# vressegu/sdeflow-light

Measured on AMD Instinct MI355X. Metric: score-matching train steps/sec (+ reverse-SDE sample steps/sec), higher is better.
Workload: dtype f32

## Files before the change

sdeflow_light_amd/csrc/conv_kernels.hip:

```cpp
#include "common.h"
#include <algorithm>
#include <type_traits>
#include <stdlib.h>

#define CONV_MAX_SRC 2

struct ConvGeom {
  int N, Hi, Wi, Ho, Wo;
  int KH, KW, strideH, padH, strideW, padW;
  int mode;
  int ups;
};

struct ConvArgs {
  ConvGeom g;
  const float* src[CONV_MAX_SRC];
  int C[CONV_MAX_SRC];
  int koff[CONV_MAX_SRC];
  int nsrc;
  const float* Wp;
  int Cout, CoutP, Ktot;
  const float* bias;
  const float* samp_bias;
  int n_bias, n_samp;
// ... 1126 lines not shown
  tile_origin<16, 16>(tile, tiles_x, tiles_y, n, y0, x0);
  auto stage = [&](int s_, int c0) __attribute__((always_inline)) {
    f32x4 st[H18_NST], ga, gb;
    unsigned valid;
    halo18_load(A, g, A.src[s_], A.C[s_], up, c0, (size_t)n * ctot_all + (s_ ? A.C[0] : 0), n, y0, x0, tid, st, valid, ga, gb);
    halo18_store(A, cur, tid, st, valid, ga, gb);
  };

  const size_t a_co_stride = (size_t)16 * A.Ktot, pos_stride = (size_t)A.CoutP * A.Ktot;
  if constexpr (WL) {
    static_assert(NCO == 2, "the LDS weight image is laid out for two output-channel tiles");
    float* wbuf = cw_lds + halo * CT_P;
    auto ngrp_of = [&](int s_, int c_) { const int rem = A.C[s_] - c_ * CT_KC; return rem >= CT_KC ? 2 : ((rem + 15) >> 4); };
    auto wfill = [&](int s_, int c_, int g_, int half, int b) __attribute__((always_inline)) {
      wino_wfill(A.Wp + (size_t)(co0 + il) * A.Ktot + A.koff[s_] + c_ * CT_KC + 16 * g_ + 4 * q + (size_t)(8 * half) * pos_stride,
                 wbuf + b * 4096, w, pos_stride, a_co_stride);
    };
    int cs = 0, cc = 0, grp = 0, step = 0;
    wfill(0, 0, 0, 0, 0);
    for (;;) {
      if (grp == 0) {
        asm volatile("s_waitcnt lgkmcnt(0)\n\ts_barrier" ::: "memory");
        stage(cs, cc * CT_KC);
      }
      int ns = cs, nc = cc, ng = grp + 1;
      bool more = true;
      if (ng >= ngrp_of(cs, cc)) {
        ng = 0; ++nc;
        if (nc >= nch[cs]) { nc = 0; ++ns; more = ns < A.nsrc; }
      }
      f32x4 d[4][4];
#pragma unroll
      for (int half = 0; half < 2; ++half) {
        asm volatile("s_waitcnt vmcnt(0) lgkmcnt(0)\n\ts_barrier" ::: "memory");
        if (half == 0) wfill(cs, cc, grp, 1, (step + 1) & 1);
        else if (more) wfill(ns, nc, ng, 0, (step + 1) & 1);
        if (half == 0) {
          wino_patch_load<HW>(d, cur + pbase + 16 * grp, tx == 7);
          wino_input_transform(d);
        }
        wino_mfma_lds<8>(acc, d, wbuf + (step & 1) * 4096 + lane * 4, 8 * half);
        ++step;
      }
      if (!more) break;
      cs = ns; cc = nc; grp = ng;
    }
  } else
  for (int cs = 0; cs < A.nsrc; ++cs)
    for (int cc = 0; cc < (cs ? nch[1] : nch[0]); ++cc) {
      asm volatile("s_waitcnt lgkmcnt(0)\n\ts_barrier" ::: "memory");
      stage(cs, cc * CT_KC);
      asm volatile("s_waitcnt lgkmcnt(0)\n\ts_barrier" ::: "memory");
      const int C = A.C[cs], c0 = cc * CT_KC;
      const int ngrp = (C - c0 >= CT_KC) ? 2 : ((C - c0 + 15) >> 4);
      const float* wbase = A.Wp + (size_t)(co0 + il) * A.Ktot + A.koff[cs] + c0 + 4 * q;
      f32x4 an[NCO];
#pragma unroll
      for (int c = 0; c < NCO; ++c) an[c] = *reinterpret_cast<const f32x4*>(wbase + c * a_co_stride);
      const float* wq = wbase;
      for (int grp = 0; grp < ngrp; ++grp) {
        f32x4 d[4][4];
        wino_patch_load<HW>(d, cur + pbase + 16 * grp, tx == 7);
        wino_input_transform(d);
        __builtin_amdgcn_sched_barrier(0);
#pragma unroll
        for (int pos = 0; pos < 16; ++pos) {
          f32x4 a[NCO];
#pragma unroll
          for (int c = 0; c < NCO; ++c) a[c] = an[c];
          if (pos < 15) wq += pos_stride;
          else wq = wbase + 16 * (grp + 1);
          asm volatile("" : "+v"(wq));
          if (pos < 15 || grp + 1 < ngrp) {
#pragma unroll
            for (int c = 0; c < NCO; ++c) an[c] = *reinterpret_cast<const f32x4*>(wq + c * a_co_stride);
          }
          const f32x4 b = d[pos >> 2][pos & 3];
#pragma unroll
          for (int r = 0; r < 4; ++r)
#pragma unroll
            for (int c = 0; c < NCO; ++c) acc[pos][c] = mfma16(a[c][r], b[r], acc[pos][c]);
          __builtin_amdgcn_sched_barrier(0);
        }
      }
    }

  wino_epilogue<NCO>(A, acc, n, y0, x0, w, co0, (tile - n * tiles_x * tiles_y) * 4 + w, lane);
}

__global__ void __launch_bounds__(256, 1) k_conv_wino_p32(ConvArgs A, int tiles_x, int tiles_y, int n_tiles) {
  extern __shared__ __attribute__((aligned(16))) float cw_lds[];
  constexpr int NCO = 2, HW = H18_HW, halo = HW * HW;
  const int tid = threadIdx.x, w = tid >> 6, lane = tid & 63, il = lane & 15, q = lane >> 4;
  const ConvGeom g = A.g;
  float* wbuf = cw_lds;
  float* hb0 = cw_lds + 2 * 16 * 2 * 256;
  float* hb1 = hb0 + halo * CT_P;
  const int tt = 16 * w + il, ty = tt >> 3, tx = tt & 7;
  const int pbase = (2 * ty * HW + 2 * tx) * CT_P + 4 * q;
  const size_t a_co_stride = (size_t)16 * A.Ktot, pos_stride = (size_t)A.CoutP * A.Ktot;
  int t = blockIdx.x;
  if (t >= n_tiles) return;
  {
    const float* src = A.Wp + (size_t)il * A.Ktot + 4 * q;
#pragma unroll
    for (int j = 0; j < 16; ++j) {
      const int pw = 16 * w + j, grp = pw >> 5, pos = (pw >> 1) & 15, c = pw & 1;
      __builtin_amdgcn_global_load_lds((const __attribute__((address_space(1))) void*)(src + (size_t)pos * pos_stride + c * a_co_stride + 16 * grp),
                                       (__attribute__((address_space(3))) void*)(wbuf + pw * 256), 16, 0, 0);
    }
  }
  const int up = g.ups ? 1 : 0;
  const int C = A.C[0];
  f32x4 st[H18_NST], ga, gb;
  unsigned valid;
  auto stage_load = [&](int tile) __attribute__((always_inline)) {
    int n, y0, x0;
    tile_origin<16, 16>(tile, tiles_x, tiles_y, n, y0, x0);
    halo18_load(A, g, A.src[0], C, up, 0, (size_t)n * C, n, y0, x0, tid, st, valid, ga, gb);
  };
  stage_load(t);
  halo18_store(A, hb0, tid, st, valid, ga, gb);
  asm volatile("s_waitcnt vmcnt(0) lgkmcnt(0)\n\ts_barrier" ::: "memory");
  float* cur = hb0;
  float* nxt = hb1;
  const int ngrp = (C + 15) >> 4;
  for (; t < n_tiles; t += gridDim.x) {
    const int tn = t + gridDim.x;
    const bool more = tn < n_tiles;
    if (more) stage_load(tn);
    f32x4 acc[16][NCO];
#pragma unroll
    for (int p = 0; p < 16; ++p)
#pragma unroll
      for (int c = 0; c < NCO; ++c) acc[p][c] = f32x4{0, 0, 0, 0};
    for (int grp = 0; grp < ngrp; ++grp) {
      f32x4 d[4][4];
#pragma unroll
      for (int i = 0; i < 4; ++i)
#pragma unroll
        for (int j = 0; j < 4; ++j) d[i][j] = *reinterpret_cast<const f32x4*>(cur + pbase + (i * HW + j) * CT_P + 16 * grp);
      wino_input_transform(d);
      wino_mfma_lds<16>(acc, d, wbuf + grp * (16 * 2 * 256) + lane * 4, 0);
    }
    int n, y0, x0;
    tile_origin<16, 16>(t, tiles_x, tiles_y, n, y0, x0);
    wino_epilogue<NCO>(A, acc, n, y0, x0, w, 0, (t - n * tiles_x * tiles_y) * 4 + w, lane);
    if (more) halo18_store(A, nxt, tid, st, valid, ga, gb);
    asm volatile("s_waitcnt lgkmcnt(0)\n\ts_barrier" ::: "memory");
    float* sw = cur; cur = nxt; nxt = sw;
  }
}

constexpr int WP_HPIECES = 21;
constexpr int WP_HSTAGE = WP_HPIECES * 64 * 4;
constexpr int WP_LDS_BYTES = (2 * 4096 + 2 * WP_HSTAGE) * (int)sizeof(float);

__global__ void __launch_bounds__(256, 2) k_conv_wino_pipe(ConvArgs A, int tiles_x, int tiles_y, int n_tiles, int n_cob) {
  extern __shared__ __attribute__((aligned(16))) float cw_lds[];
  constexpr int NCO = 2, HW = 18;
  const int tid = threadIdx.x, lane = tid & 63, il = lane & 15, q = lane >> 4;
  const int w = __builtin_amdgcn_readfirstlane(tid >> 6);
  const ConvGeom g = A.g;
  float* wbuf = cw_lds;
  float* hbuf = cw_lds + 2 * 4096;
  const int xcd = blockIdx.x & 7, loc_stride = gridDim.x >> 3;
  int loc = blockIdx.x >> 3;
  int tile = (loc / n_cob) * 8 + xcd, cob = loc % n_cob;
  if (tile >= n_tiles) return;
  const int ngrp = A.Ktot >> 4, tpi = tiles_x * tiles_y, up = g.ups ? 1 : 0;
  const size_t a_co_stride = (size_t)16 * A.Ktot, pos_stride = (size_t)A.CoutP * A.Ktot;
  const int tt = 16 * w + il, ty = tt >> 3, tx = tt & 7;
  const int P0 = 2 * ty * HW + 2 * tx, h0 = (P0 >> 1) & 3;

  auto wfill = [&](int cob_, int grp_, int half) __attribute__((always_inline)) {
    wino_wfill(A.Wp + (size_t)(cob_ * (NCO * 16) + il) * A.Ktot + 16 * grp_ + 4 * q + (size_t)(8 * half) * pos_stride,
               wbuf + half * 4096, w, pos_stride, a_co_stride);
  };
  const int Hu = g.Hi << up, Wu = g.Wi << up;
  int hpk[(WP_HPIECES + 3) / 4];
#pragma unroll
  for (int j = 0; j < (WP_HPIECES + 3) / 4; ++j) {
    const int sl = 64 * (w + 4 * j) + lane, P = sl >> 2, c = (sl & 3) ^ ((P >> 1) & 3), hy = P / HW, hx = P - hy * HW;
    hpk[j] = P < HW * HW ? (hy << 16) | (hx << 2) | c : 0x7fff << 16;
  }
  auto hfill = [&](int tile_, int grp_, int b) __attribute__((always_inline)) {
    const int n = tile_ / tpi, r = tile_ - n * tpi, ty_i = r / tiles_x, y0 = ty_i * 16, x0 = (r - ty_i * tiles_x) * 16;
    const bool s1 = 16 * grp_ >= A.C[0];
    const int C = s1 ? A.C[1] : A.C[0];
    const float* base = (s1 ? A.src[1] : A.src[0]) + (size_t)n * g.Hi * g.Wi * C + (16 * grp_ - (s1 ? A.C[0] : 0));
#pragma unroll
    for (int j = 0; j < (WP_HPIECES + 3) / 4; ++j) {
      const int m = w + 4 * j;
      if (m < WP_HPIECES) {
        int pk = hpk[j];
        asm volatile("" : "+v"(pk));
        const int c = pk & 3, iy = y0 + (pk >> 16) - 1, ix = x0 + ((pk >> 2) & 31) - 1;
        const bool in = (unsigned)iy < (unsigned)Hu && (unsigned)ix < (unsigned)Wu;
        const float* p = in ? base + (((iy >> up) * g.Wi + (ix >> up)) * C + 4 * c) : g_wino_zero;
        __builtin_amdgcn_global_load_lds((const __attribute__((address_space(1))) void*)p,
                                         (__attribute__((address_space(3))) void*)(hbuf + b * WP_HSTAGE + m * 256), 16, 0, 0);
      }
    }
  };

  f32x4 acc[16][NCO];
#pragma unroll
  for (int p = 0; p < 16; ++p)
#pragma unroll
    for (int c = 0; c < NCO; ++c) acc[p][c] = f32x4{0, 0, 0, 0};
  int grp = 0, hb = 0;
  wfill(cob, 0, 0);
  hfill(tile, 0, 0);
  for (;;) {
    int nloc = loc, ntile = tile, ncob = cob, ngrp_ = grp + 1;
    if (ngrp_ == ngrp) {
      ngrp_ = 0; nloc = loc + loc_stride;
      ntile = (nloc / n_cob) * 8 + xcd; ncob = nloc % n_cob;
    }
    const bool more = ntile < n_tiles;
    f32x4 d[4][4];
#pragma unroll
    for (int half = 0; half < 2; ++half) {
      if (half == 1 && more) asm volatile("s_waitcnt vmcnt(5) lgkmcnt(0)\n\ts_barrier" ::: "memory");
      else asm volatile("s_waitcnt vmcnt(0) lgkmcnt(0)\n\ts_barrier" ::: "memory");
      if (half == 0) {
        wfill(cob, grp, 1);
        if (more) hfill(ntile, ngrp_, hb ^ 1);
      } else if (more) {
        wfill(ncob, ngrp_, 0);
      }
      if (half == 0) {
        const float* hs = hbuf + hb * WP_HSTAGE;
#pragma unroll
        for (int i = 0; i < 4; ++i) {
          const float* rp = hs + 16 * (P0 + i * HW) + 4 * (q ^ ((h0 + i) & 3));
          d[i][0] = *reinterpret_cast<const f32x4*>(rp);
          d[i][1] = *reinterpret_cast<const f32x4*>(rp + 16);
        }
#pragma unroll
        for (int i = 0; i < 4; ++i)
#pragma unroll
          for (int j = 0; j < 2; ++j)
#pragma unroll
            for (int r = 0; r < 4; ++r) d[i][2 + j][r] = dpp_from_next_lane(d[i][j][r]);
        if (tx == 7) {
#pragma unroll
          for (int i = 0; i < 4; ++i) {
            const float* rp = hs + 16 * (P0 + i * HW + 2) + 4 * (q ^ ((h0 + i + 1) & 3));
            d[i][2] = *reinterpret_cast<const f32x4*>(rp);
            d[i][3] = *reinterpret_cast<const f32x4*>(rp + 16);
          }
        }
        wino_input_transform(d);
      }
      const float* wb = wbuf + half * 4096 + lane * 4;
      f32x4 a0 = *reinterpret_cast<const f32x4*>(wb), a1 = *reinterpret_cast<const f32x4*>(wb + 256);
#pragma unroll
      for (int pl = 0; pl < 8; ++pl) {
        const f32x4 x0_ = a0, x1_ = a1;
        if (pl < 7) {
          a0 = *reinterpret_cast<const f32x4*>(wb + (2 * pl + 2) * 256);
          a1 = *reinterpret_cast<const f32x4*>(wb + (2 * pl + 3) * 256);
        }
        const int pos = 8 * half + pl;
        const f32x4 b = d[pos >> 2][pos & 3];
#pragma unroll
        for (int r = 0; r < 4; ++r) {
          acc[pos][0] = mfma16(x0_[r], b[r], acc[pos][0]);
          acc[pos][1] = mfma16(x1_[r], b[r], acc[pos][1]);
        }
        __builtin_amdgcn_sched_barrier(0);
      }
    }
    if (ngrp_ == 0) {
      const int n = tile / tpi, r = tile - n * tpi, ty_i = r / tiles_x;
      wino_epilogue<NCO>(A, acc, n, ty_i * 16, (r - ty_i * tiles_x) * 16, w, cob * (NCO * 16), r * 4 + w, lane);
      if (!more) break;
#pragma unroll
      for (int p = 0; p < 16; ++p)
#pragma unroll
        for (int c = 0; c < NCO; ++c) acc[p][c] = f32x4{0, 0, 0, 0};
    }
    loc = nloc; tile = ntile; cob = ncob; grp = ngrp_; hb ^= 1;
  }
}

__global__ void __launch_bounds__(256) k_wino_pack_batched(const msgm_pack_job_t* __restrict__ jobs) {
  const msgm_pack_job_t J = jobs[blockIdx.y];
  const int64_t tot = (int64_t)J.rows * J.ncols;
  for (int64_t e = blockIdx.x * (int64_t)blockDim.x + threadIdx.x; e < tot; e += (int64_t)gridDim.x * blockDim.x) {
    const int c = (int)(e % J.ncols), r = (int)(e / J.ncols);
    const float* w = J.W + r * J.sr + (J.col_off + c) * J.sc;
    float gk[3][3], h[4][3];
#pragma unroll
    for (int t = 0; t < 9; ++t) gk[t / 3][t % 3] = w[t * J.st];
#pragma unroll
    for (int j = 0; j < 3; ++j) {
      h[0][j] = gk[0][j];
      h[1][j] = 0.5f * (gk[0][j] + gk[1][j] + gk[2][j]);
      h[2][j] = 0.5f * (gk[0][j] - gk[1][j] + gk[2][j]);
      h[3][j] = gk[2][j];
    }
#pragma unroll
    for (int i = 0; i < 4; ++i) {
      const float u0 = h[i][0], u1 = 0.5f * (h[i][0] + h[i][1] + h[i][2]), u2 = 0.5f * (h[i][0] - h[i][1] + h[i][2]), u3 = h[i][2];
      float* p = J.Wp + ((int64_t)(4 * i) * J.rowsP + r) * J.Ktot + J.kp_off + c;
      const int64_t ps = (int64_t)J.rowsP * J.Ktot;
      p[0] = u0; p[ps] = u1; p[2 * ps] = u2; p[3 * ps] = u3;
    }
  }
}

struct WgradArgs {
  ConvGeom g;
  const float* gy;
  const float* src;
  int C, koff;
  float* dWp;
  int Cout, CoutP, Ktot;
  int chunk;
  float* dbias;
  int n_bias;
  unsigned short tm_c[16], tm_o[16];
  float* slab; long slab_stride;
};

constexpr int WT_GP = 132;
#define WT_SWZ(ch) ((((ch) >> 2) & 7) << 2)
__host__ __device__ constexpr int wt_kw(int TH, int TAPS) { return TH == 1 ? TAPS : (TAPS == 9 ? 3 : 1); }
__host__ __device__ constexpr int wt_halo(int TH, int TW, int KH, int KW) { return (TH + KH - 1) * (TW + KW - 1); }
__host__ __device__ constexpr int wt_in_pitch(int halo) { return ((halo + 2) & ~7) + 5; }
__host__ __device__ constexpr int wt_buf_floats(int in_pitch) { return 32 * WT_GP + 32 * in_pitch; }
__host__ __device__ constexpr int wt_tile_bufs(int TAPS) { return TAPS == 9 ? 2 : 1; }

struct WgradShare { int coblk, cblk, co0, c0, t_beg, t_end; };
__device__ __forceinline__ WgradShare wgrad_share(const WgradArgs& A, int tiles_per_wg, int n_tiles) {
  const int cblocks = (A.C + 31) / 32;
  const int coblk = blockIdx.y / cblocks, cblk = blockIdx.y - coblk * cblocks;
  const int t_beg = blockIdx.x * tiles_per_wg;
  return WgradShare{coblk, cblk, coblk * 32, cblk * 32, t_beg, min(t_beg + tiles_per_wg, n_tiles)};
}

template <int TH, int TW, int KH, int KW, bool RAG, int MAXIN>
__device__ __forceinline__ void wtile_load(const WgradArgs& A, int tile, int tiles_x, int tiles_y, int co0, int c0, int tid,
                                           f32x4 (&sg)[4], f32x4 (&si)[MAXIN]) {
  constexpr int HW = TW + KW - 1, n_in = wt_halo(TH, TW, KH, KW) * 8;
  const ConvGeom& g = A.g;
  const int up = g.ups ? 1 : 0;
  int n, y0, x0;
  tile_origin<TH, TW>(tile, tiles_x, tiles_y, n, y0, x0);
#pragma unroll
  for (int k = 0; k < 4; ++k) {
    const int idx = tid + 256 * k;
    const int p = idx >> 3, c4 = idx & 7;
    const int py = p / TW, px = p - py * TW;
    const int oy = y0 + py, ox = x0 + px, co = co0 + 4 * c4;
    f32x4 v = {0, 0, 0, 0};
    if (oy < g.Ho && ox < g.Wo && co < A.Cout) {
      const float* gp = A.gy + (((size_t)n * g.Ho + oy) * g.Wo + ox) * A.Cout + co;
      if (!RAG) v = *reinterpret_cast<const f32x4*>(gp);
      else {
#pragma unroll
        for (int r = 0; r < 4; ++r) if (co + r < A.Cout) v[r] = gp[r];
      }
    }
    sg[k] = v;
  }
#pragma unroll
  for (int k = 0; k < MAXIN; ++k) {
    const int idx = tid + 256 * k;
    f32x4 v = {0, 0, 0, 0};
    if (idx < n_in) {
      const int hp = idx >> 3, c4 = idx & 7;
      const int hy = hp / HW, hx = hp - hy * HW;
      const int iy = y0 + hy - g.padH, ix = x0 + hx - g.padW, c = c0 + 4 * c4;
      if (iy >= 0 && iy < (g.Hi << up) && ix >= 0 && ix < (g.Wi << up) && c < A.C) {
        const float* sp = A.src + (((size_t)n * g.Hi + (iy >> up)) * g.Wi + (ix >> up)) * A.C + c;
        if (!RAG) v = *reinterpret_cast<const f32x4*>(sp);
        else {
#pragma unroll
          for (int r = 0; r < 4; ++r) if (c + r < A.C) v[r] = sp[r];
        }
      }
    }
    si[k] = v;
  }
}

__device__ __forceinline__ void wgrad_bias_add(const float* gT, int tid, float& bsum) {
  const float* gr = gT + (tid >> 3) * WT_GP + 16 * (tid & 7);
  f32x4 t4 = *reinterpret_cast<const f32x4*>(gr);
  t4 += *reinterpret_cast<const f32x4*>(gr + 4);
  t4 += *reinterpret_cast<const f32x4*>(gr + 8);
  t4 += *reinterpret_cast<const f32x4*>(gr + 12);
  bsum += (t4[0] + t4[1]) + (t4[2] + t4[3]);
}
__device__ __forceinline__ void wgrad_bias_store(const WgradArgs& A, float bsum, int tid, int co0, int taps) {
  bsum += __shfl_xor(bsum, 1, 64);
  bsum += __shfl_xor(bsum, 2, 64);
  bsum += __shfl_xor(bsum, 4, 64);
  const int co = co0 + (tid >> 3);
  if ((tid & 7) == 0 && co < A.Cout) A.slab[(size_t)blockIdx.x * A.slab_stride + (size_t)taps * A.CoutP * A.C + co] = bsum;
}

__device__ __forceinline__ void wgrad_slab_store(const WgradArgs& A, int tap, int co_base, int q, int c, f32x4 v) {
#pragma unroll
  for (int r = 0; r < 4; ++r) {
    const int co = co_base + 4 * q + r;
    if (co < A.Cout && c < A.C) A.slab[(size_t)blockIdx.x * A.slab_stride + (size_t)(tap * A.CoutP + co) * A.C + c] = v[r];
  }
}

template <int MT, int KT>
__global__ void __launch_bounds__(256) k_conv_wgrad(WgradArgs A) {
  __shared__ float red[4][MT * KT * 256];
  const int tid = threadIdx.x, w = tid >> 6, lane = tid & 63, il = lane & 15, q = lane >> 4;
  const ConvGeom g = A.g;
  const int HoWo = g.Ho * g.Wo;
  const int Mtot = g.N * HoWo;
  const int cblocks = (A.C + 16 * KT - 1) / (16 * KT);
  const int coblk = blockIdx.y / cblocks, cblk = blockIdx.y - coblk * cblocks;
  const int co0 = coblk * 16 * MT, c0 = cblk * 16 * KT;
// ... 799 lines not shown
    const int mid = (lo + hi + 1) >> 1;
    if (jobs[mid].block_begin <= blk) lo = mid; else hi = mid - 1;
  }
  const msgm_reduce_job_t J = jobs[lo];
  slot_reduce_block(blk - J.block_begin, J.part, J.nslots, (long)J.stride, (long)J.n_elem, J.out, J.C, J.Ktot, J.koff, J.accumulate,
                    J.rowsP, J.rows, (long)J.n_elem2, J.out2);
}

__global__ void __launch_bounds__(256) k_colsum(const float* __restrict__ x, float* __restrict__ S, int P, int C, int chunk) {
  __shared__ float red[256];
  const int n = blockIdx.x;
  const float* xn = x + (size_t)n * P * C;
  const int p0 = blockIdx.y * chunk, p1 = min(p0 + chunk, P);
  for (int cb = 0; cb < C; cb += 256) {
    const int lanes_c = min(C - cb, 256);
    const int rows = 256 / lanes_c;
    const int c = threadIdx.x % lanes_c, pr = threadIdx.x / lanes_c;
    float s = 0.f;
    if (pr < rows)
      for (int p = p0 + pr; p < p1; p += rows) s += xn[(size_t)p * C + cb + c];
    red[threadIdx.x] = (pr < rows) ? s : 0.f;
    __syncthreads();
    if (pr == 0) {
      float t = 0.f;
      for (int r = 0; r < rows; ++r) t += red[r * lanes_c + c];
      S[((size_t)blockIdx.y * gridDim.x + n) * C + cb + c] = t;
    }
    __syncthreads();
  }
}

__global__ void k_add_row(float* __restrict__ x, const float* __restrict__ E, int N, int P, int C, int pos, float sgn) {
  const int64_t tot = (int64_t)N * C;
  for (int64_t e = blockIdx.x * (int64_t)blockDim.x + threadIdx.x; e < tot; e += (int64_t)gridDim.x * blockDim.x) {
    const int n = (int)(e / C), c = (int)(e - (int64_t)n * C);
    x[((size_t)n * P + pos) * C + c] += sgn * E[e];
  }
}

__global__ void k_gather_row(const float* __restrict__ x, float* __restrict__ out, int N, int P, int C, int pos) {
  const int64_t tot = (int64_t)N * C;
  for (int64_t e = blockIdx.x * (int64_t)blockDim.x + threadIdx.x; e < tot; e += (int64_t)gridDim.x * blockDim.x) {
    const int n = (int)(e / C), c = (int)(e - (int64_t)n * C);
    out[e] = x[((size_t)n * P + pos) * C + c];
  }
}

static int check_geom(const msgm_conv_geom_t* g) {
  if (!g || g->N <= 0 || g->Hi <= 0 || g->Wi <= 0 || g->Ho <= 0 || g->Wo <= 0 || g->KH <= 0 || g->KW <= 0 ||
      g->strideH <= 0 || g->padH < 0 || g->strideW <= 0 || g->padW < 0 || (g->mode != 0 && g->mode != 1) ||
      (g->ups != 0 && g->ups != 1))
    return MSGM_E_BADARG;
  if ((int64_t)g->N * g->Ho * g->Wo >= (1ll << 31) || (int64_t)g->N * g->Hi * g->Wi >= (1ll << 31)) return MSGM_E_UNSUPPORTED;
  return MSGM_OK;
}
static ConvGeom to_geom(const msgm_conv_geom_t* g) {
  return ConvGeom{g->N, g->Hi, g->Wi, g->Ho, g->Wo, g->KH, g->KW, g->strideH, g->padH, g->strideW, g->padW, g->mode, g->ups};
}

static bool conv_same(const msgm_conv_geom_t* g) {
  const int ups_sh = g->ups ? 1 : 0;
  return g->strideH == 1 && g->strideW == 1 && (g->Hi << ups_sh) == g->Ho && (g->Wi << ups_sh) == g->Wo &&
         (g->KH & 1) && (g->KW & 1) && g->KH <= 3 && g->KW <= 3 && g->padH == (g->KH - 1) / 2 && g->padW == (g->KW - 1) / 2;
}

static int conv_n_cu() {
  static const int n_cu = [] { int d = 0, n = 256; (void)hipGetDevice(&d); (void)hipDeviceGetAttribute(&n, hipDeviceAttributeMultiprocessorCount, d); return n > 0 ? n : 256; }();
  return n_cu;
}
template <auto K, int BYTES = 160 * 1024>
static void conv_raise_lds_limit() {
  static const int once = [] {
    (void)hipFuncSetAttribute(reinterpret_cast<const void*>(K), hipFuncAttributeMaxDynamicSharedMemorySize, BYTES);
    return 0;
  }();
  (void)once;
}

extern "C" {

static bool conv_tile_eligible(const msgm_conv_geom_t* geom, int32_t C0, bool has1, int32_t C1, int32_t CoutP) {
  const bool fast = (C0 % 16 == 0) && (!has1 || C1 % 16 == 0);
  return conv_same(geom) && (!geom->ups || geom->mode == 0) && fast && CoutP % 32 == 0 && (int64_t)geom->Ho * geom->Wo >= 64 &&
         (geom->Ho > 1 ? geom->KH == geom->KW : geom->KH == 1);
}

static bool conv_wino_eligible(const msgm_conv_geom_t* geom, int32_t C0, int32_t C1, int32_t CoutP, int cmul) {
  return geom->mode == 0 && geom->KH == 3 && geom->KW == 3 && conv_same(geom) && geom->Ho % 16 == 0 && geom->Wo % 16 == 0 &&
         C0 % cmul == 0 && C1 % cmul == 0 && CoutP % 32 == 0;
}

int msgm_conv_wino_supported(const msgm_conv_geom_t* geom, int32_t C0, int32_t C1, int32_t CoutP) {
  if (check_geom(geom)) return 0;
  return conv_wino_eligible(geom, C0, C1, CoutP, 16) ? 1 : 0;
}

static int conv_args(ConvArgs* A, const msgm_conv_geom_t* geom, const float* src0, int32_t C0, const float* src1, int32_t C1,
                     const void* W, int32_t Cout, int32_t CoutP, int32_t Ktot, const float* bias, const float* samp_bias,
                     int32_t n_bias, int32_t n_samp, float* out, int32_t accumulate, const msgm_conv_fuse_t* fuse,
                     bool padded_k) {
  int rc = check_geom(geom);
  if (rc) return rc;
  if (fuse && ((fuse->in_scale == nullptr) != (fuse->in_shift == nullptr) || (fuse->in_act != 0 && fuse->in_act != 1)))
    return MSGM_E_BADARG;
  if (!src0 || !W || !out || C0 <= 0 || Cout <= 0 || (src1 && C1 <= 0)) return MSGM_E_BADARG;
  const int k0 = padded_k ? ((C0 + 15) / 16) * 16 : C0, k1 = !src1 ? 0 : padded_k ? ((C1 + 15) / 16) * 16 : C1;
  if (Ktot != k0 + k1 || CoutP % 16 || CoutP < Cout) return MSGM_E_BADARG;
  *A = ConvArgs{};
  A->g = to_geom(geom);
  A->src[0] = src0; A->C[0] = C0; A->koff[0] = 0;
  A->src[1] = src1; A->C[1] = src1 ? C1 : 0; A->koff[1] = k0;
  A->nsrc = src1 ? 2 : 1;
  A->Wp = static_cast<const float*>(W); A->Cout = Cout; A->CoutP = CoutP; A->Ktot = Ktot;
  A->bias = bias; A->samp_bias = samp_bias; A->n_bias = n_bias; A->n_samp = n_samp; A->out = out; A->accumulate = accumulate;
  if (fuse) {
    A->residual = fuse->residual; A->in_scale = fuse->in_scale; A->in_shift = fuse->in_shift; A->in_act = fuse->in_act;
    for (int i = 0; i < 16; ++i) A->tapmask_in[i] = fuse->tapmask_in[i];
    for (int i = 0; i < 8; ++i) A->tapmask_out[i] = fuse->tapmask_out[i];
    A->cstat = fuse->chanstats;
  }
  return MSGM_OK;
}
static bool conv_has_masks(const ConvArgs& A) {
  unsigned m = 0;
  for (int i = 0; i < 16; ++i) m |= A.tapmask_in[i];
  for (int i = 0; i < 8; ++i) m |= A.tapmask_out[i];
  return m != 0;
}

int msgm_wino_pack_weights_batched(const msgm_pack_job_t* jobs, int32_t n_jobs, msgm_stream_t stream) {
  if (!jobs || n_jobs <= 0) return MSGM_E_BADARG;
  hipLaunchKernelGGL(k_wino_pack_batched, dim3(8, (unsigned)n_jobs), dim3(256), 0, S(stream), jobs);
  return msgm_check_launch();
}

static bool tile16_chanstats(ConvArgs& A) {
  if (!A.cstat) return true;
  A.cs_S = (A.g.Wo / 16) * (A.g.Ho / 16) * 4;
  return A.Cout % 4 == 0;
}

int msgm_conv_forward_wino(const msgm_conv_geom_t* geom, const float* src0, int32_t C0, const float* src1, int32_t C1,
                           const float* WpW, int32_t Cout, int32_t CoutP, int32_t Ktot, const float* bias,
                           const float* samp_bias, int32_t n_bias, int32_t n_samp, float* out, int32_t accumulate,
                           const msgm_conv_fuse_t* fuse, msgm_stream_t stream) {
  ConvArgs A;
  int rc = conv_args(&A, geom, src0, C0, src1, C1, WpW, Cout, CoutP, Ktot, bias, samp_bias, n_bias, n_samp, out, accumulate,
                     fuse, true);
  if (rc) return rc;
  if (!conv_wino_eligible(geom, C0, A.C[1], CoutP, 16) || !tile16_chanstats(A)) return MSGM_E_UNSUPPORTED;
  const int tiles_x = geom->Wo / 16, tiles_y = geom->Ho / 16;
  const int n_tiles = tiles_x * tiles_y * geom->N, gy = CoutP / 32;
  if (!A.in_scale) {
    conv_raise_lds_limit<&k_conv_wino_pipe, WP_LDS_BYTES>();
    const int items_per_xcd = gy * ((n_tiles + 7) / 8);
    const int wg_per_xcd = std::min(items_per_xcd, std::max(1, 2 * conv_n_cu() / 8));
    hipLaunchKernelGGL(k_conv_wino_pipe, dim3((unsigned)(8 * wg_per_xcd)), dim3(256), WP_LDS_BYTES, S(stream), A, tiles_x, tiles_y, n_tiles, gy);
    return msgm_check_launch();
  }
  const size_t lds = (size_t)18 * 18 * CT_P * sizeof(float);
  dim3 grid((unsigned)(8 * gy * ((n_tiles + 7) / 8)));
  constexpr int p32_min = 1024;
  if (!src1 && Ktot == 32 && CoutP == 32 && n_tiles >= p32_min) {
    conv_raise_lds_limit<&k_conv_wino_p32>();
    const size_t lds32 = ((size_t)2 * 16 * 2 * 256 + 2 * 18 * 18 * CT_P) * sizeof(float);
    hipLaunchKernelGGL(k_conv_wino_p32, dim3((unsigned)conv_n_cu()), dim3(256), lds32, S(stream), A, tiles_x, tiles_y, n_tiles);
    return msgm_check_launch();
  }
  if (Ktot < 64) {
    hipLaunchKernelGGL((k_conv_wino<2, false>), grid, dim3(256), lds, S(stream), A, tiles_x, tiles_y, n_tiles, gy);
    return msgm_check_launch();
  }
  conv_raise_lds_limit<&k_conv_wino<2, true>>();
  hipLaunchKernelGGL((k_conv_wino<2, true>), grid, dim3(256), lds + 2 * 4096 * sizeof(float), S(stream), A, tiles_x, tiles_y, n_tiles, gy);
  return msgm_check_launch();
}

__global__ void __launch_bounds__(256) k_b6_split(const float* __restrict__ Wp, __bf16* __restrict__ Wb, long n) {
  for (long e = (long)blockIdx.x * 256 + threadIdx.x; e < n; e += (long)gridDim.x * 256) {
    const float x = Wp[e];
    const __bf16 h = (__bf16)x;
    const float r1 = x - (float)h;
    const __bf16 m = (__bf16)r1;
    Wb[e] = h; Wb[n + e] = m; Wb[2 * n + e] = (__bf16)(r1 - (float)m);
  }
}

int msgm_conv_b6_supported(const msgm_conv_geom_t* geom, int32_t C0, int32_t C1, int32_t CoutP) {
  if (check_geom(geom)) return 0;
  return conv_wino_eligible(geom, C0, C1, CoutP, 32) ? 1 : 0;
}

int msgm_b6_split_weights(const float* Wp, void* Wb, int64_t n_elem, msgm_stream_t stream) {
  if (!Wp || !Wb || n_elem <= 0) return MSGM_E_BADARG;
  hipLaunchKernelGGL(k_b6_split, dim3((unsigned)grid_for(n_elem, 256, 2048)), dim3(256), 0, S(stream), Wp, static_cast<__bf16*>(Wb), (long)n_elem);
  return msgm_check_launch();
}

int msgm_conv_forward_b6(const msgm_conv_geom_t* geom, const float* src0, int32_t C0, const float* src1, int32_t C1,
                         const void* Wb, int32_t Cout, int32_t CoutP, int32_t Ktot, const float* bias,
                         const float* samp_bias, int32_t n_bias, int32_t n_samp, float* out, int32_t accumulate,
                         const msgm_conv_fuse_t* fuse, msgm_stream_t stream) {
  ConvArgs A;
  int rc = conv_args(&A, geom, src0, C0, src1, C1, Wb, Cout, CoutP, Ktot, bias, samp_bias, n_bias, n_samp, out, accumulate,
                     fuse, false);
  if (rc) return rc;
  if (!conv_wino_eligible(geom, C0, A.C[1], CoutP, 32) || conv_has_masks(A) || !tile16_chanstats(A)) return MSGM_E_UNSUPPORTED;
  const int nco = (CoutP % 64 == 0) ? 4 : 2;
  const int tiles_x = (geom->Wo + 15) / 16, tiles_y = (geom->Ho + 15) / 16;
  const int n_tiles = tiles_x * tiles_y * geom->N, gy = CoutP / (16 * nco);
  int per = (int)(((int64_t)n_tiles * gy) / (512 * 8));
  if (per > 4) per = 4;
  if (per < 1) per = 1;
  const int n_tgrp = (n_tiles + per - 1) / per;
  dim3 grid((unsigned)(8 * gy * ((n_tgrp + 7) / 8)));
  const size_t lds = (size_t)18 * 18 * 52 * sizeof(float);
  conv_raise_lds_limit<&k_conv_tile<16, 16, 4, 3, 4, false, true>>();
  conv_raise_lds_limit<&k_conv_tile<16, 16, 2, 3, 4, false, true>>();
  if (nco == 4) hipLaunchKernelGGL((k_conv_tile<16, 16, 4, 3, 4, false, true>), grid, dim3(256), lds, S(stream), A, 0, tiles_x, tiles_y, per, n_tiles, gy, n_tgrp);
  else hipLaunchKernelGGL((k_conv_tile<16, 16, 2, 3, 4, false, true>), grid, dim3(256), lds, S(stream), A, 0, tiles_x, tiles_y, per, n_tiles, gy, n_tgrp);
  return msgm_check_launch();
}

struct ConvRoute {
  int kind;
  int pt, kg;
  bool wide, two_d; int nco, TH, TW, tiles_x, tiles_y;
};
static bool conv_small_shape(const msgm_conv_geom_t* geom, bool has1, bool masks) {
  return conv_same(geom) && geom->KH == 3 && geom->KW == 3 && !geom->ups && geom->Ho > 1 && !has1 && !masks;
}
static bool conv_dgrad_s2_shape(const msgm_conv_geom_t* geom, int32_t C0, bool has1, int32_t Cout, int32_t CoutP, bool masks) {
  return geom->mode == 1 && geom->KH == 3 && geom->KW == 3 && geom->strideH == 2 && geom->strideW == 2 && geom->padH == 1 &&
         geom->padW == 1 && !geom->ups && geom->Ho == 2 * geom->Hi && geom->Wo == 2 * geom->Wi && !has1 && !masks &&
         C0 % 32 == 0 && Cout % 32 == 0 && CoutP == Cout;
}
static ConvRoute conv_route(const msgm_conv_geom_t* geom, int32_t C0, bool has1, int32_t C1, int32_t Cout, int32_t CoutP,
                            bool masks, bool both_extra = false , bool any_size = false) {
  ConvRoute r{};
  const int64_t Mtot = (int64_t)geom->N * geom->Ho * geom->Wo;
  if (conv_dgrad_s2_shape(geom, C0, has1, Cout, CoutP, masks)) { r.kind = 5; return r; }
  if (conv_small_shape(geom, has1, masks)) {
    if (C0 <= 4 && Cout == 32 && CoutP == 32) { r.kind = 3; return r; }
    if (C0 == 32 && Cout <= 4 && geom->mode == 0) { r.kind = 4; return r; }
  }
  const bool fast = (C0 % 16 == 0) && (!has1 || C1 % 16 == 0);
  const int Ktot = ((C0 + 15) / 16) * 16 + (has1 ? ((C1 + 15) / 16) * 16 : 0);
  const int kg = Ktot / 16;
  if (conv_same(geom) && geom->KH == 1 && geom->KW == 1 && !geom->ups && fast && !masks && (Mtot >= 4096 || any_size) &&
      (kg == 2 || kg == 4 || kg == 6 || kg == 8 || kg == 12 || kg == 16) && Cout % 16 == 0 && !both_extra) {
    const int pt = kg <= 4 ? 4 : (kg <= 8 ? 2 : (kg == 12 && (geom->Ho * geom->Wo) % 32 == 0 ? 2 : 1));
    if ((geom->Ho * geom->Wo) % (16 * pt) == 0) { r.kind = 1; r.kg = kg; r.pt = pt; return r; }
  }
  if (conv_tile_eligible(geom, C0, has1, C1, CoutP)) {
    r.kind = 2;
    r.two_d = geom->Ho > 1;
    r.nco = (CoutP % 64 == 0) ? 4 : 2;
    bool wide = geom->KW == 3 && (r.two_d ? (geom->Ho >= 16 && geom->Wo >= 16) : geom->Wo >= 256);
    if (wide) {
      const int64_t wtiles = (int64_t)geom->N * ((geom->Wo + (r.two_d ? 15 : 255)) / (r.two_d ? 16 : 256)) *
                             (r.two_d ? (geom->Ho + 15) / 16 : 1) * (CoutP / (16 * r.nco));
      if (wtiles < 512) wide = false;
    }
    r.wide = wide;
    r.TH = r.two_d ? (wide ? 16 : 8) : 1; r.TW = r.two_d ? 16 : (wide ? 256 : 128);
    r.tiles_x = (geom->Wo + r.TW - 1) / r.TW; r.tiles_y = (geom->Ho + r.TH - 1) / r.TH;
    if (!wide && r.nco == 4 && !masks && (int64_t)geom->N * r.tiles_x * r.tiles_y * (CoutP / 64) < 512) r.nco = 2;
    return r;
  }
  r.pt = (CoutP >= 64 && CoutP % 64 == 0) ? 2 : 4;
  return r;
}
static int conv_route_slots(const ConvRoute& r, const msgm_conv_geom_t* geom, int32_t Cout) {
  if (Cout % 4) return 0;
  if (r.kind == 1) { const int P = geom->Ho * geom->Wo; return P % (16 * r.pt) == 0 ? P / (16 * r.pt) : 0; }
  if (r.kind == 2) return r.tiles_x * r.tiles_y * 4;
  if (r.kind == 3) { const int P = geom->Ho * geom->Wo; return P % 64 == 0 ? P / 64 : 0; }
  if (r.kind == 4 || r.kind == 5) return 0;
  const int P = geom->Ho * geom->Wo, px = 16 * r.pt;
  return P % px == 0 ? P / px : 0;
}

int32_t msgm_conv_chanstats_slots(const msgm_conv_geom_t* geom, int32_t C0, int32_t C1, int32_t Cout, int32_t CoutP) {
  if (check_geom(geom) || C0 <= 0 || C1 < 0 || Cout <= 0 || CoutP < Cout || CoutP % 16) return 0;
  return conv_route_slots(conv_route(geom, C0, C1 > 0, C1, Cout, CoutP, false), geom, Cout);
}

static bool conv_in_transform_ok(const ConvRoute& r, const msgm_conv_geom_t* geom, int32_t C0, bool has1, int32_t C1, int32_t CoutP) {
  return r.kind == 4 || conv_tile_eligible(geom, C0, has1, C1, CoutP);
}

int msgm_conv_input_transform_supported(const msgm_conv_geom_t* geom, int32_t C0, int32_t C1, int32_t Cout, int32_t CoutP) {
  if (check_geom(geom)) return 0;
  return conv_in_transform_ok(conv_route(geom, C0, C1 > 0, C1, Cout, CoutP, false), geom, C0, C1 > 0, C1, CoutP) ? 1 : 0;
}

int msgm_conv_forward(const msgm_conv_geom_t* geom, const float* src0, int32_t C0, const float* src1, int32_t C1,
                      const float* Wp, int32_t Cout, int32_t CoutP, int32_t Ktot, const float* bias,
                      const float* samp_bias, int32_t n_bias, int32_t n_samp, float* out, int32_t accumulate,
                      msgm_stream_t stream) {
  return msgm_conv_forward_fused(geom, src0, C0, src1, C1, Wp, Cout, CoutP, Ktot, bias, samp_bias, n_bias, n_samp, out,
                                 accumulate, nullptr, stream);
}

int msgm_conv_forward_fused(const msgm_conv_geom_t* geom, const float* src0, int32_t C0, const float* src1, int32_t C1,
                            const float* Wp, int32_t Cout, int32_t CoutP, int32_t Ktot, const float* bias,
// ... 445 lines not shown
```

Before: 10.21.

## Use buffer loads to LDS and interleave Winograd transform with MFMAs in pipe kernel

Result: faster. 10.36, median of 6 (+1.5%).

```diff
diff --git a/sdeflow_light_amd/csrc/conv_kernels.hip b/sdeflow_light_amd/csrc/conv_kernels.hip
--- a/sdeflow_light_amd/csrc/conv_kernels.hip
+++ b/sdeflow_light_amd/csrc/conv_kernels.hip
@@ -1302,6 +1302,10 @@
   }
 }
 
+__device__ __forceinline__ void wino_row_transform(f32x4 (&x)[4]) {
+  const f32x4 c0_ = x[0] - x[2], c1_ = x[1] + x[2], c2_ = x[2] - x[1], c3_ = x[1] - x[3];
+  x[0] = c0_; x[1] = c1_; x[2] = c2_; x[3] = c3_;
+}
 constexpr int WP_HPIECES = 21;
 constexpr int WP_HSTAGE = WP_HPIECES * 64 * 4;
 constexpr int WP_LDS_BYTES = (2 * 4096 + 2 * WP_HSTAGE) * (int)sizeof(float);
@@ -1323,34 +1327,46 @@
   const int tt = 16 * w + il, ty = tt >> 3, tx = tt & 7;
   const int P0 = 2 * ty * HW + 2 * tx, h0 = (P0 >> 1) & 3;
 
+  const __amdgpu_buffer_rsrc_t wrs = __builtin_amdgcn_make_buffer_rsrc((void*)A.Wp, 0, 16 * (int)pos_stride * 4, 0x00020000);
+  const int wlane = (il * A.Ktot + 4 * q) * 4;
   auto wfill = [&](int cob_, int grp_, int half) __attribute__((always_inline)) {
-    wino_wfill(A.Wp + (size_t)(cob_ * (NCO * 16) + il) * A.Ktot + 16 * grp_ + 4 * q + (size_t)(8 * half) * pos_stride,
-               wbuf + half * 4096, w, pos_stride, a_co_stride);
+    const int so = ((cob_ * (NCO * 16)) * A.Ktot + 16 * grp_ + (8 * half + 2 * w) * (int)pos_stride) * 4;
+#pragma unroll
+    for (int j = 0; j < 4; ++j) {
+      const int pw = 4 * w + j;
+      __builtin_amdgcn_raw_ptr_buffer_load_lds(wrs, (__attribute__((address_space(3))) void*)(wbuf + half * 4096 + pw * 256), 16, wlane,
+                                               so + ((j >> 1) * (int)pos_stride + (j & 1) * (int)a_co_stride) * 4, 0, 0);
+    }
   };
   const int Hu = g.Hi << up, Wu = g.Wi << up;
-  int hpk[(WP_HPIECES + 3) / 4];
-#pragma unroll
-  for (int j = 0; j < (WP_HPIECES + 3) / 4; ++j) {
-    const int sl = 64 * (w + 4 * j) + lane, P = sl >> 2, c = (sl & 3) ^ ((P >> 1) & 3), hy = P / HW, hx = P - hy * HW;
-    hpk[j] = P < HW * HW ? (hy << 16) | (hx << 2) | c : 0x7fff << 16;
-  }
-  auto hfill = [&](int tile_, int grp_, int b) __attribute__((always_inline)) {
+  int hoff[(WP_HPIECES + 3) / 4];
+  const float* hbase;
+  int hnum, hsub;
+  auto hsetup = [&](int tile_, int s1) __attribute__((always_inline)) {
     const int n = tile_ / tpi, r = tile_ - n * tpi, ty_i = r / tiles_x, y0 = ty_i * 16, x0 = (r - ty_i * tiles_x) * 16;
-    const bool s1 = 16 * grp_ >= A.C[0];
     const int C = s1 ? A.C[1] : A.C[0];
-    const float* base = (s1 ? A.src[1] : A.src[0]) + (size_t)n * g.Hi * g.Wi * C + (16 * grp_ - (s1 ? A.C[0] : 0));
+    hbase = (s1 ? A.src[1] : A.src[0]) + (size_t)n * g.Hi * g.Wi * C;
+    hnum = g.Hi * g.Wi * C * 4;
+    hsub = s1 ? 4 * A.C[0] : 0;
+    int l = lane;
+    asm volatile("" : "+v"(l));
+#pragma unroll
+    for (int j = 0; j < (WP_HPIECES + 3) / 4; ++j) {
+      const int sl = 64 * (w + 4 * j) + l, P = sl >> 2, c = (sl & 3) ^ ((P >> 1) & 3), hy = P / HW, hx = P - hy * HW;
+      const int iy = y0 + hy - 1, ix = x0 + hx - 1;
+      const bool in = P < HW * HW && (unsigned)iy < (unsigned)Hu && (unsigned)ix < (unsigned)Wu;
+      hoff[j] = in ? (((iy >> up) * g.Wi + (ix >> up)) * C + 4 * c) * 4 : (int)0x80000000;
+    }
+  };
+  auto hfill = [&](int grp_, int b) __attribute__((always_inline)) {
+    const __amdgpu_buffer_rsrc_t rs = __builtin_amdgcn_make_buffer_rsrc((void*)hbase, 0, hnum, 0x00020000);
+    const int soff = 64 * grp_ - hsub;
 #pragma unroll
     for (int j = 0; j < (WP_HPIECES + 3) / 4; ++j) {
       const int m = w + 4 * j;
-      if (m < WP_HPIECES) {
-        int pk = hpk[j];
-        asm volatile("" : "+v"(pk));
-        const int c = pk & 3, iy = y0 + (pk >> 16) - 1, ix = x0 + ((pk >> 2) & 31) - 1;
-        const bool in = (unsigned)iy < (unsigned)Hu && (unsigned)ix < (unsigned)Wu;
-        const float* p = in ? base + (((iy >> up) * g.Wi + (ix >> up)) * C + 4 * c) : g_wino_zero;
-        __builtin_amdgcn_global_load_lds((const __attribute__((address_space(1))) void*)p,
-                                         (__attribute__((address_space(3))) void*)(hbuf + b * WP_HSTAGE + m * 256), 16, 0, 0);
-      }
+      if (j < WP_HPIECES / 4 || m < WP_HPIECES)
+        __builtin_amdgcn_raw_ptr_buffer_load_lds(rs, (__attribute__((address_space(3))) void*)(hbuf + b * WP_HSTAGE + m * 256), 16,
+                                                 hoff[j], soff, 0, 0);
     }
   };
 
@@ -1361,25 +1377,25 @@
     for (int c = 0; c < NCO; ++c) acc[p][c] = f32x4{0, 0, 0, 0};
   int grp = 0, hb = 0;
   wfill(cob, 0, 0);
-  hfill(tile, 0, 0);
+  hsetup(tile, 0);
+  hfill(0, 0);
   for (;;) {
     int nloc = loc, ntile = tile, ncob = cob, ngrp_ = grp + 1;
-    if (ngrp_ == ngrp) {
+    const bool last = ngrp_ == ngrp;
+    if (last) {
       ngrp_ = 0; nloc = loc + loc_stride;
-      ntile = (nloc / n_cob) * 8 + xcd; ncob = nloc % n_cob;
+      asm volatile("" : "+s"(nloc));
+      const int nq = nloc / n_cob;
+      ntile = nq * 8 + xcd; ncob = nloc - nq * n_cob;
     }
     const bool more = ntile < n_tiles;
-    f32x4 d[4][4];
+    f32x4 d[4][4], t1[4];
 #pragma unroll
     for (int half = 0; half < 2; ++half) {
       if (half == 1 && more) asm volatile("s_waitcnt vmcnt(5) lgkmcnt(0)\n\ts_barrier" ::: "memory");
       else asm volatile("s_waitcnt vmcnt(0) lgkmcnt(0)\n\ts_barrier" ::: "memory");
-      if (half == 0) {
-        wfill(cob, grp, 1);
-        if (more) hfill(ntile, ngrp_, hb ^ 1);
-      } else if (more) {
-        wfill(ncob, ngrp_, 0);
-      }
+      const float* wb = wbuf + half * 4096 + lane * 4;
+      f32x4 a0, a1;
       if (half == 0) {
         const float* hs = hbuf + hb * WP_HSTAGE;
 #pragma unroll
@@ -1388,6 +1404,15 @@
           d[i][0] = *reinterpret_cast<const f32x4*>(rp);
           d[i][1] = *reinterpret_cast<const f32x4*>(rp + 16);
         }
+        a0 = *reinterpret_cast<const f32x4*>(wb); a1 = *reinterpret_cast<const f32x4*>(wb + 256);
+        __builtin_amdgcn_sched_barrier(0);
+        wfill(cob, grp, 1);
+        if (more) {
+          if (last) hsetup(ntile, 0);
+          else if (16 * ngrp_ == A.C[0]) hsetup(tile, 1);
+          hfill(ngrp_, hb ^ 1);
+        }
+        __builtin_amdgcn_sched_barrier(0);
 #pragma unroll
         for (int i = 0; i < 4; ++i)
 #pragma unroll
@@ -1402,10 +1427,17 @@
             d[i][3] = *reinterpret_cast<const f32x4*>(rp + 16);
           }
         }
-        wino_input_transform(d);
-      }
-      const float* wb = wbuf + half * 4096 + lane * 4;
-      f32x4 a0 = *reinterpret_cast<const f32x4*>(wb), a1 = *reinterpret_cast<const f32x4*>(wb + 256);
+#pragma unroll
+        for (int j = 0; j < 4; ++j) {
+          t1[j] = d[1][j] + d[2][j];
+          d[0][j] = d[0][j] - d[2][j];
+        }
+        wino_row_transform(d[0]);
+        wino_row_transform(t1);
+      } else {
+        a0 = *reinterpret_cast<const f32x4*>(wb); a1 = *reinterpret_cast<const f32x4*>(wb + 256);
+        if (more) wfill(ncob, ngrp_, 0);
+      }
 #pragma unroll
       for (int pl = 0; pl < 8; ++pl) {
         const f32x4 x0_ = a0, x1_ = a1;
@@ -1414,11 +1446,21 @@
           a1 = *reinterpret_cast<const f32x4*>(wb + (2 * pl + 3) * 256);
         }
         const int pos = 8 * half + pl;
-        const f32x4 b = d[pos >> 2][pos & 3];
+        const f32x4 b = half ? d[pos >> 2][pos & 3] : pl < 4 ? d[0][pl] : t1[pl - 4];
 #pragma unroll
         for (int r = 0; r < 4; ++r) {
           acc[pos][0] = mfma16(x0_[r], b[r], acc[pos][0]);
           acc[pos][1] = mfma16(x1_[r], b[r], acc[pos][1]);
+        }
+        if (half == 0) {
+          if (pl < 4) {
+            d[3][pl] = d[1][pl] - d[3][pl];
+            d[2][pl] = d[2][pl] - d[1][pl];
+            asm volatile("" : "+v"(d[3][pl]), "+v"(d[2][pl]));
+          } else if (pl < 6) {
+            wino_row_transform(d[pl - 2]);
+            asm volatile("" : "+v"(d[pl - 2][0]), "+v"(d[pl - 2][1]), "+v"(d[pl - 2][2]), "+v"(d[pl - 2][3]));
+          }
         }
         __builtin_amdgcn_sched_barrier(0);
       }
@@ -2524,6 +2566,8 @@
   const int tiles_x = geom->Wo / 16, tiles_y = geom->Ho / 16;
   const int n_tiles = tiles_x * tiles_y * geom->N, gy = CoutP / 32;
   if (!A.in_scale) {
+    const int64_t lim = (int64_t)1 << 31;
+    if ((int64_t)geom->Hi * geom->Wi * std::max(C0, A.C[1]) * 4 >= lim || (int64_t)16 * CoutP * Ktot * 4 >= lim) return MSGM_E_UNSUPPORTED;
     conv_raise_lds_limit<&k_conv_wino_pipe, WP_LDS_BYTES>();
     const int items_per_xcd = gy * ((n_tiles + 7) / 8);
     const int wg_per_xcd = std::min(items_per_xcd, std::max(1, 2 * conv_n_cu() / 8));
```
